# submarine0418/underwater_image_enhancement

Hardware: AMD Instinct MI355X
Metric: megapixels/sec enhanced (higher is better)
Workload: dtype f32/f64

## Files before the change

### include/uwie.h

```cpp
#ifndef UWIE_H_
#define UWIE_H_

#include <stddef.h>
#include <stdint.h>

#ifdef __cplusplus
extern "C" {
#endif

#define UWIE_OK 0
#define UWIE_E_INVALID (-1)
#define UWIE_E_WORKSPACE (-2)
#define UWIE_E_HIP (-3)
#define UWIE_E_NODEVICE (-4)
#define UWIE_E_DEVICE (-5)

#define UWIE_SURFACE_SIX 0
#define UWIE_SURFACE_DICT 1

#define UWIE_DICT_STRONG_DEHAZING 0
#define UWIE_DICT_MEDIUM_DEHAZING 1
#define UWIE_DICT_LIGHT_ENHANCEMENT 2
#define UWIE_DICT_CLAHE_ENHANCEMENT 3
#define UWIE_DICT_HISTOGRAM_EQUALIZATION 4
// ... 280 lines not shown
                           size_t workspace_bytes, void *stream);

int uwie_transmission_init(uwie_ctx *ctx, const uint8_t *d_in, const int32_t *d_kind, const float *d_A, int batch,
                           int H, int W, const uwie_params *p, float *d_t0, uint8_t *d_gray, void *stream);

int uwie_dark_patch_plan(int H, int W, int k, int *tile_w, int *tile_h);

int uwie_box_filter_f64(uwie_ctx *ctx, const double *d_src, double *d_dst, int batch, int H, int W, int ksize,
                        void *d_workspace, size_t workspace_bytes, void *stream);

int uwie_guided_filter(uwie_ctx *ctx, const uint8_t *d_gray, const float *d_t0, int batch, int H, int W, int ksize,
                       double eps, int exact, double *d_t, void *d_workspace, size_t workspace_bytes, void *stream);

int uwie_guided_plan(int batch, int H, int W, int ksize, int *split_row0, int *split_rows);

int uwie_guided_fill(int batch, int H, int W, int ksize, long long *items);

typedef struct uwie_clahe_plan_info {
    int32_t tile_w, tile_h, padded, clip_limit, wide_lut, nchunk, cells_walk, cells_flat;
} uwie_clahe_plan_info;
int uwie_clahe_plan(int batch, int H, int W, int tiles_x, int tiles_y, double clip_limit, int recomputed,
                    uwie_clahe_plan_info *out);

int uwie_restore(uwie_ctx *ctx, const uint8_t *d_in, const int32_t *d_kind, const float *d_A, const double *d_t,
                 int batch, int H, int W, float *d_out_f32, void *stream);

int uwie_percentiles_f32(uwie_ctx *ctx, const float *d_img, int batch, int H, int W, const double *q_percent, int nq,
                         float *d_out, void *d_workspace, size_t workspace_bytes, void *stream);

int uwie_percentiles_f64(uwie_ctx *ctx, const double *d_img, int batch, int H, int W, const double *q_percent, int nq,
                         double *d_out, void *d_workspace, size_t workspace_bytes, void *stream);

int uwie_stretch_f32(uwie_ctx *ctx, const float *d_img, float *d_out, int batch, int H, int W, double lo_percent,
                     double hi_percent, void *d_workspace, size_t workspace_bytes, void *stream);

int uwie_gamma_f32(uwie_ctx *ctx, const float *d_img, float *d_out, size_t n, double g, int mode, void *stream);

int uwie_clahe_f32(uwie_ctx *ctx, const float *d_img, float *d_out, int batch, int H, int W, double clip_limit,
                   int tiles_x, int tiles_y, void *d_workspace, size_t workspace_bytes, void *stream);

int uwie_rgb2gray_u8(uwie_ctx *ctx, const uint8_t *d_rgb, uint8_t *d_gray, size_t npixels, int gray_shift,
                     void *stream);
int uwie_rgb2lab_u8(uwie_ctx *ctx, const uint8_t *d_rgb, uint8_t *d_lab, size_t npixels, void *stream);
int uwie_lab2rgb_u8(uwie_ctx *ctx, const uint8_t *d_lab, uint8_t *d_rgb, size_t npixels, void *stream);
int uwie_clahe_u8(uwie_ctx *ctx, const uint8_t *d_plane, uint8_t *d_out, int batch, int H, int W, double clip_limit,
                  int tiles_x, int tiles_y, void *d_workspace, size_t workspace_bytes, void *stream);
// ... 10 lines not shown
```

### underwater_image_enhancement_amd/_lib.py

```python
from __future__ import annotations

import ctypes
import os
import subprocess

_HERE = os.path.dirname(os.path.abspath(__file__))
LIB_PATH = os.path.join(_HERE, "lib", "libuwie.so")
CSRC = os.path.join(_HERE, "csrc")

SURFACE_SIX, SURFACE_DICT = 0, 1
STATUS_DIFF_RANK = 16
STATUS_CLASSIFY_NAN = 64
LOSS_IDENTITY, LOSS_VGG, LOSS_GATED = 0, 1, 2
VGG_F32, VGG_F16, VGG_PARAMS = 0, 1, 1735488
PARAM_NET_PARAMS = {True: 8500100, False: 8459652}
MASKS_GIVEN, MASKS_DRAWN = 0, 1
TRAINER_PARAMS, TRAINER_GRADS, TRAINER_EXP_AVG, TRAINER_EXP_AVG_SQ = 0, 1, 2, 3
FLIP_LR, FLIP_UD = 1, 2
RESIZE_MAX_SIDE, RESIZE_MAX_SRC = 4096, 32768
INTER_F64, INTER_FX32, INTER_F32T = 0, 1, 2
DICT_STRATEGIES = {
    "strong_dehazing": 0,
    "medium_dehazing": 1,
    "light_enhancement": 2,
# ... 114 lines not shown
    "uwie_last_error": [],
    "uwie_version": [],
    "uwie_create": [_I, ctypes.POINTER(_VP)],
    "uwie_destroy": [_VP],
    "uwie_device_status": [_VP, _VP, ctypes.POINTER(ctypes.c_uint32)],
    "uwie_profile_enable": [_VP, _I],
    "uwie_profile_filter": [_VP, ctypes.c_char_p],
    "uwie_profile_collect": [_VP],
    "uwie_profile_row": [_VP, _I, ctypes.POINTER(ctypes.c_char_p), ctypes.POINTER(_D), ctypes.POINTER(_I)],
    "uwie_params_init": [_PP, _I, _I],
    "uwie_set_tuning": [_VP, ctypes.c_char_p, _I],
    "uwie_get_tuning": [_VP, ctypes.c_char_p, ctypes.POINTER(_I)],
    "uwie_workspace_bytes": [_I, _I, _I, _PP],
    "uwie_workspace_bytes_ctx": [_VP, _I, _I, _I, _PP],
    "uwie_workspace_bytes_all": [_I, _I, _I, _VP],
    "uwie_workspace_bytes_float": [_I, _I, _I, _PP, _I],
    "uwie_enhance_f32": [_VP, _VP, _VP, _VP, _VP, _I, _I, _I, _PP, _VP, _SZ, _VP],
    "uwie_enhance_f64": [_VP, _VP, _VP, _VP, _I, _I, _I, _PP, _VP, _SZ, _VP],
    "uwie_cast_classify_f32": [_VP, _VP, _I, _I, _I, _VP, _VP, _VP],
    "uwie_color_correct_f32": [_VP, _VP, _VP, _VP, _I, _I, _I, _VP],
    "uwie_guided_plan": [_I, _I, _I, _I, ctypes.POINTER(ctypes.c_int), ctypes.POINTER(ctypes.c_int)],
    "uwie_guided_fill": [_I, _I, _I, _I, ctypes.POINTER(ctypes.c_longlong)],
    "uwie_clahe_plan": [_I, _I, _I, _I, _I, _D, _I, ctypes.POINTER(UwieClahePlan)],
    "uwie_dark_patch_plan": [_I, _I, _I, ctypes.POINTER(ctypes.c_int), ctypes.POINTER(ctypes.c_int)],
    "uwie_enhance_u8": [_VP, _VP, _VP, _VP, _I, _I, _I, _PP, _VP, _SZ, _VP],
    "uwie_enhance_u8_f64": [_VP, _VP, _VP, _VP, _I, _I, _I, _PP, _VP, _SZ, _VP],
    "uwie_enhance_percentiles": [_VP, _VP, _SZ, _I, _I, _I, _PP, _VP, _VP],
    "uwie_enhance_all_u8": [_VP, _VP, _VP, _VP, _I, _I, _I, _VP, _VP, _SZ, _VP],
    "uwie_workspace_bytes_select": [_I, _I, _I, _VP, _I, _I],
    "uwie_select_best_u8": [_VP, _VP, _I, _I, _I, _VP, _I, _VP, _VP, _VP, _VP, _VP, _VP, _SZ, _VP],
    "uwie_workspace_bytes_underwater": [_I, _I, _I],
    "uwie_underwater_plan": [_I, _I, ctypes.POINTER(ctypes.c_int), ctypes.POINTER(ctypes.c_int)],
    "uwie_underwater_scores_u8": [_VP, _VP, _I, _I, _I, _I, _VP, _VP, _SZ, _VP],
    "uwie_workspace_bytes_reference": [_I, _I, _I],
    "uwie_reference_plan": [_I, _I, ctypes.POINTER(ctypes.c_int), ctypes.POINTER(ctypes.c_int)],
    "uwie_reference_scores_u8": [_VP, _VP, _VP, _I, _I, _I, _I, _I, _VP, _VP, _SZ, _VP],
    "uwie_workspace_bytes_gray_world": [_I, _I, _I],
    "uwie_gray_world_plan": [_I, _I, ctypes.POINTER(ctypes.c_int), ctypes.POINTER(ctypes.c_int)],
    "uwie_gray_world_u8": [_VP, _VP, _I, _I, _I, _D, _D, _D, _VP, _VP, _VP, _SZ, _VP],
    "uwie_workspace_bytes_fusion": [_I, _I, _I, _I],
    "uwie_fusion_plan": [_I, _I, _I, ctypes.POINTER(ctypes.c_int), ctypes.POINTER(ctypes.c_int)],
    "uwie_fusion_table": [_D, ctypes.POINTER(ctypes.c_uint8)],
    "uwie_fusion_u8": [_VP, _VP, _I, _I, _I, _D, _I, _I, _VP, _VP, _VP, _VP, _VP, _SZ, _VP],
    "uwie_pick_best_u8": [_VP, _VP, _I, _I, _I, _I, _VP, _I, _I, _VP, _VP, _VP],
    "uwie_diff_enhance_f32": [_VP, _VP, _VP, _I, _I, _I, _I, _VP, _I, _VP, _SZ, _VP],
    "uwie_diff_enhance_save_f32": [_VP, _VP, _VP, _I, _I, _I, _I, _VP, _I, _VP, _VP, _SZ, _VP],
# ... 134 lines not shown
```

### underwater_image_enhancement_amd/csrc/api.hip

```cpp
#include <algorithm>
#include <cmath>
#include <cstdarg>
#include <cstdio>
#include <cstring>
#include <type_traits>

#include "common.h"

#include <cstdlib>

namespace uwie {

static thread_local char g_err[512] = "";
static thread_local uwie_ctx *g_ctx = nullptr;
static const Tuning g_default_tuning{};

const Tuning &tune() { return g_ctx ? g_ctx->tune : g_default_tuning; }
uwie_ctx *current_ctx() { return g_ctx; }

void set_error(const char *fmt, ...)
{
    va_list ap;
    va_start(ap, fmt);
    vsnprintf(g_err, sizeof g_err, fmt, ap);
// ... 2016 lines not shown
    *items = g.route == GF_SPLIT ? guided_items(s, g) : 0;
    return UWIE_OK;
}

int uwie_dark_patch_plan(int H, int W, int k, int *tile_w, int *tile_h)
{
    UWIE_REQUIRE(tile_w && tile_h, "dark_patch_plan: NULL pointer");
    UWIE_CHECK_SHAPE(1, H, W);
    UWIE_REQUIRE(k >= 0 && k <= 31, "dark_patch_plan: dark_patch must be 0 .. 31");
    dark_patch_tile(tile_w, tile_h);
    return UWIE_OK;
}

int uwie_clahe_plan(int batch, int H, int W, int tiles_x, int tiles_y, double clip_limit, int recomputed,
                    uwie_clahe_plan_info *out)
{
    UWIE_REQUIRE(out, "clahe_plan: NULL pointer");
    UWIE_CHECK_SHAPE(batch, H, W);
    UWIE_REQUIRE(tiles_x >= 1 && tiles_y >= 1 && tiles_x * tiles_y <= 4096, "clahe_plan: bad tile grid");
    clahe_plan_info(Shape{batch, H, W}, clip_limit, tiles_x, tiles_y, recomputed != 0, out);
    return UWIE_OK;
}

int uwie_restore(uwie_ctx *ctx, const uint8_t *d_in, const int32_t *d_kind, const float *d_A, const double *d_t,
                 int batch, int H, int W, float *d_out_f32, void *stream)
{
    UWIE_REQUIRE(ctx && d_in && d_A && d_t && d_out_f32, "restore: NULL pointer");
    UWIE_SCOPE(ctx);
    UWIE_CHECK_SHAPE(batch, H, W);
    return launch_restore(d_in, d_kind, d_A, d_t, Shape{batch, H, W}, d_out_f32, (hipStream_t)stream);
}

int uwie_percentiles_f32(uwie_ctx *ctx, const float *d_img, int batch, int H, int W, const double *q_percent, int nq,
                         float *d_out, void *d_workspace, size_t workspace_bytes, void *stream)
{
    UWIE_REQUIRE(ctx && d_img && q_percent && d_out, "percentiles: NULL pointer");
    UWIE_SCOPE(ctx);
    UWIE_CHECK_SHAPE(batch, H, W);
    const Shape s{batch, H, W};
    UWIE_CHECK_WS(select_ws_bytes(s));
    return launch_percentiles(d_img, 0, s, q_percent, nq, d_out, d_workspace, (hipStream_t)stream);
}

int uwie_percentiles_f64(uwie_ctx *ctx, const double *d_img, int batch, int H, int W, const double *q_percent, int nq,
                         double *d_out, void *d_workspace, size_t workspace_bytes, void *stream)
{
// ... 129 lines not shown
```

### underwater_image_enhancement_amd/csrc/common.h

```cpp
#pragma once
#include <hip/hip_runtime.h>
#include <stddef.h>
#include <stdint.h>

#include "../../include/uwie.h"

namespace uwie {

void set_error(const char *fmt, ...);
#define UWIE_HIP_CHECK(expr)                                                            \
    do {                                                                                \
        hipError_t _e = (expr);                                                         \
        if (_e != hipSuccess) {                                                         \
            ::uwie::set_error("%s failed: %s (%s:%d)", #expr, hipGetErrorString(_e), __FILE__, __LINE__); \
            return UWIE_E_HIP;                                                          \
        }                                                                               \
    } while (0)
#define UWIE_LAUNCH_CHECK() UWIE_HIP_CHECK(hipGetLastError())
#define UWIE_REQUIRE(cond, msg)                 \
    do {                                        \
        if (!(cond)) {                          \
            ::uwie::set_error("%s", msg);       \
            return UWIE_E_INVALID;              \
        }                                       \
    } while (0)

constexpr int kCastBinadeMin = -2;
constexpr int kCastBinades = 34;

struct LabTables {
    uint16_t gamma[256];
    uint16_t cbrt[3072];
    int32_t fwd[9];
    uint8_t invgamma[4096];
    int32_t ltoyf[512];
    int32_t abtoxz[36864];
    int32_t inv[9];
};

struct CastTables {
    uint32_t R[kCastBinades][256];
    uint8_t tie[kCastBinades][256];
    uint32_t RT[256][kCastBinades];
    uint2 RT2[128][kCastBinades];
    uint8_t tiebin[256];
};

void build_lab_tables(LabTables *t);
void build_cast_tables(CastTables *t);

struct Profiler;
Profiler *prof_create();
void prof_destroy(Profiler *p);
void prof_enable(Profiler *p, bool on);
void prof_filter(Profiler *p, const char *name);
void prof_bind(Profiler *p);
int prof_collect(Profiler *p);
int prof_row(Profiler *p, int i, const char **name, double *ms, int *calls);
class ProfScope {
public:
// ... 457 lines not shown
```

### underwater_image_enhancement_amd/csrc/k_fused.hip

```cpp
#include <cstdlib>

#include "common.h"
#include "devutil.h"
#include "restore.h"

namespace uwie {

namespace {


typedef float f32x2 __attribute__((ext_vector_type(2)));
#ifndef UWIE_CLAHE_PREFETCH
#define UWIE_CLAHE_PREFETCH 0
#endif
#ifndef UWIE_STRETCH_WAVES
#define UWIE_STRETCH_WAVES 5
#endif
#define UWIE_DESCALE(x, n) (((x) + (1 << ((n)-1))) >> (n))

template <bool LIN, bool COLLECT, int NW = 2, typename V = float>
__global__ void __launch_bounds__(256) k_restore_planar_hist(RestoreSrc S, int npx, V *__restrict__ planar,
                                                             uint32_t *__restrict__ ghist, LinState *__restrict__ lin,
                                                             V *__restrict__ lists, uint32_t cap)
{
    constexpr int NB = LIN ? 2052 : 2048;
    constexpr bool F64 = sizeof(V) == 8;
    constexpr bool FAST = LIN && !F64;
    constexpr int NS = COLLECT ? 3 * NW : 1, SN = COLLECT ? (NW == 2 && !F64 ? 256 : 128) : 1;
    __shared__ uint32_t h[3][NB];
    __shared__ V stg[NS][SN];
    __shared__ uint32_t scount[NS], sbase[NS];
    __shared__ double dtab[FAST ? 768 : 1];
    const int b = blockIdx.y, tid = threadIdx.x;
    if (ghist) {
// ... 744 lines not shown
__device__ __forceinline__ int ab_to_xz(int i)
{
    const int t = __mul24(i, 108);
    const uint32_t tp = (uint32_t)(t + ((t >> 31) & 840) + 841 * 1100);
    const int lin = (int)__umulhi(tp, 5106980u) - (1100 + 290);
    const uint32_t sq = __umul24((uint32_t)i, (uint32_t)i) >> 14;
    const int cub = (int)(__umul24(sq, (uint32_t)i) >> 14);
    return i <= 3390 ? lin : cub;
}
__device__ __forceinline__ int ab_to_xz_cubic(int i)
{
    const uint32_t sq = __umul24((uint32_t)i, (uint32_t)i) >> 14;
    return (int)(__umul24(sq, (uint32_t)i) >> 14);
}

#define UWIE_APPLY_WALKS(gpr, rstep) ((gpr) <= 256 && (rstep) * (gpr) * 8 >= 256 * 7)
constexpr bool clahe_apply_walks(int gpr) { return UWIE_APPLY_WALKS(gpr, 256 / (gpr > 1 ? gpr : 1)); }
static_assert(clahe_apply_walks(1) && clahe_apply_walks(45) && clahe_apply_walks(85), "walk: narrow cells");
static_assert(!clahe_apply_walks(86) && !clahe_apply_walks(90) && !clahe_apply_walks(111), "flat: 341 .. 444 px");
static_assert(clahe_apply_walks(112) && clahe_apply_walks(128), "walk: 445 .. 512 px");
static_assert(!clahe_apply_walks(129) && !clahe_apply_walks(223), "flat: 513 .. 892 px");
static_assert(clahe_apply_walks(224) && clahe_apply_walks(256) && !clahe_apply_walks(257), "walk up to 1024 px, flat beyond");

template <bool CODES, bool F32OUT>
__global__ void __launch_bounds__(256) k_clahe_apply_out(const LabTables *__restrict__ T, const uint8_t *__restrict__ lab,
                                                         const uint8_t *__restrict__ lut, ClaheGeom g, int nchunk,
                                                         int gamma_mode, float gexp, const uint8_t *__restrict__ fin_code,
                                                         const float *__restrict__ fin_val, uint8_t *__restrict__ out_u8,
                                                         float *__restrict__ out_f32, uint8_t *__restrict__ codes_out,
                                                         uint32_t *__restrict__ hist)
{
    constexpr int NF = CODES ? 768 : 256;
    constexpr bool TWOSTEP = CODES || F32OUT;
    constexpr int BASE = 1 << 14;
    __shared__ __attribute__((aligned(16))) int s_l[256][4];
    __shared__ int s_l2[256];
    __shared__ uint8_t s_invgamma[TWOSTEP ? 4096 : 1];
    __shared__ uint8_t s_fin[TWOSTEP ? 1 : 4096];
    __shared__ float s_ff[NF];
    __shared__ uint8_t s_fu[NF];
    __shared__ uint32_t s_h[CODES ? 4 * 768 : 1];
    __shared__ uint32_t s_lut4[4][256];
    const int tid = threadIdx.x, b = blockIdx.y;
    const int cell = blockIdx.x / nchunk, chunk = blockIdx.x - cell * nchunk;
    const int cyi = cell / (g.tx + 1), cxi = cell - cyi * (g.tx + 1);
    const int cx0 = max(cxi * g.tw - g.tw / 2, 0), cx1 = min((cxi + 1) * g.tw - g.tw / 2, g.W);
    const int ry0 = max(cyi * g.th - g.th / 2, 0), ry1 = min((cyi + 1) * g.th - g.th / 2, g.H);
    const int rows_per = (ry1 - ry0 + nchunk - 1) / nchunk;
    const int cy0 = ry0 + chunk * rows_per, cy1 = min(cy0 + rows_per, ry1);
    if (cx0 >= cx1 || cy0 >= cy1) return;
    const int wx0 = min(max(cxi - 2, 0), max(g.tx - 4, 0)), wy0 = min(max(cyi - 2, 0), max(g.ty - 4, 0));
    const int m0 = T->inv[0], m1 = T->inv[1], m2 = T->inv[2], m3 = T->inv[3], m4 = T->inv[4], m5 = T->inv[5], m6 = T->inv[6],
              m7 = T->inv[7], m8 = T->inv[8];
    {
        const int yy = T->ltoyf[2 * tid], ify = T->ltoyf[2 * tid + 1];
        *reinterpret_cast<int4 *>(&s_l[tid][0]) = make_int4(ify - 128 * BASE / 500, ify + (128 * BASE / 200 - 1), m1 * yy + (1 << 13), m4 * yy + (1 << 13));
        s_l2[tid] = m7 * yy + (1 << 13);
    }
    if (TWOSTEP)
        for (int i = tid; i < 4096; i += 256) s_invgamma[i] = T->invgamma[i];
    if (CODES) {
        for (int i = tid; i < 768; i += 256) {
            s_fu[i] = fin_code ? fin_code[(size_t)b * 768 + i] : (uint8_t)0;
            s_ff[i] = fin_val ? fin_val[(size_t)b * 768 + i] : 0.f;
        }
        if (hist)
            for (int i = tid; i < 4 * 768; i += 256) s_h[i] = 0;
    } else {
        const float y = final_value(tid, gamma_mode, gexp);
        s_ff[tid] = y;
        s_fu[tid] = (uint8_t)quant_u8(y);
    }
    const uint8_t *Lt = lut + (size_t)b * g.tx * g.ty * 256;
    {
        const int wy = tid >> 6, q = tid & 63;
        const int tyy = min(wy0 + wy, g.ty - 1);
        uint32_t d[4];
#pragma unroll
        for (int wx = 0; wx < 4; ++wx)
            d[wx] = reinterpret_cast<const uint32_t *>(Lt + (size_t)(tyy * g.tx + min(wx0 + wx, g.tx - 1)) * 256)[q];
#pragma unroll
        for (int k = 0; k < 4; ++k)
            s_lut4[wy][4 * q + k] = ((d[0] >> (8 * k)) & 255u) | (((d[1] >> (8 * k)) & 255u) << 8) | (((d[2] >> (8 * k)) & 255u) << 16) |
                                    (((d[3] >> (8 * k)) & 255u) << 24);
    }
    __syncthreads();
    if (!TWOSTEP) {
        for (int i = tid; i < 1024; i += 256) {
            const uint32_t q = reinterpret_cast<const uint32_t *>(T->invgamma)[i];
            reinterpret_cast<uint32_t *>(s_fin)[i] = (uint32_t)s_fu[q & 255] | ((uint32_t)s_fu[(q >> 8) & 255] << 8) |
                                                     ((uint32_t)s_fu[(q >> 16) & 255] << 16) | ((uint32_t)s_fu[q >> 24] << 24);
        }
        __syncthreads();
    }
    const float inv_tw = 1.0f / (float)g.tw, inv_th = 1.0f / (float)g.th;
    const int gpr = (cx1 - cx0 + 3) / 4, total = (cy1 - cy0) * gpr;
    const uint32_t gmagic = (uint32_t)(((1ull << 32) + gpr - 1) / gpr);
    struct Cols {
        uint32_t sel[4];
        float xa[4], xa1[4];
    };
    auto cols_of = [&](int x0) {
        Cols C;
#pragma unroll
        for (int i = 0; i < 4; ++i) {
            const int x = min(x0 + i, g.W - 1);
            const float txf = (float)x * inv_tw - 0.5f;
            int tx1 = (int)floorf(txf);
            int tx2 = tx1 + 1;
            C.xa[i] = txf - (float)tx1;
            C.xa1[i] = 1.0f - C.xa[i];
            tx1 = max(tx1, 0);
            tx2 = min(tx2, g.tx - 1);
            const uint32_t c1 = (uint32_t)min(max(tx1 - wx0, 0), 3), c2 = (uint32_t)min(max(tx2 - wx0, 0), 3);
            C.sel[i] = c1 | ((4u + c1) << 8) | (c2 << 16) | ((4u + c2) << 24);
        }
        return C;
    };
    auto fetch = [&](int row, int xg, uint32_t (&w)[3]) {
        const int y = cy0 + row, x0 = cx0 + 4 * xg;
        if (row < cy1 - cy0 && x0 + 4 <= cx1) {
            const u32_unaligned *q = reinterpret_cast<const u32_unaligned *>(lab + (((size_t)b * g.H + y) * g.W + x0) * 3);
            w[0] = q[0]; w[1] = q[1]; w[2] = q[2];
        }
    };
    auto group = [&](int row, int xg, const Cols &C, const uint32_t (&pre)[3], bool has_pre) {
        const int y = cy0 + row, x0 = cx0 + 4 * xg, n = min(4, cx1 - x0);
        const size_t pix = ((size_t)b * g.H + y) * g.W + x0;
        Px4 in4;
        if (n == 4) {
            uint32_t w0 = pre[0], w1 = pre[1], w2 = pre[2];
            if (!has_pre) {
                const u32_unaligned *w = reinterpret_cast<const u32_unaligned *>(lab + pix * 3);
                w0 = w[0]; w1 = w[1]; w2 = w[2];
            }
            in4.r[0] = w0 & 255; in4.g[0] = (w0 >> 8) & 255; in4.b[0] = (w0 >> 16) & 255;
            in4.r[1] = w0 >> 24; in4.g[1] = w1 & 255; in4.b[1] = (w1 >> 8) & 255;
            in4.r[2] = (w1 >> 16) & 255; in4.g[2] = w1 >> 24; in4.b[2] = w2 & 255;
            in4.r[3] = (w2 >> 8) & 255; in4.g[3] = (w2 >> 16) & 255; in4.b[3] = w2 >> 24;
        } else {
            in4 = load_px4(lab + pix * 3, n, false);
        }
        const float tyf = (float)y * inv_th - 0.5f;
        int ty1 = (int)floorf(tyf);
        int ty2 = ty1 + 1;
        const float ya = tyf - (float)ty1, ya1 = 1.0f - ya;
        ty1 = max(ty1, 0);
        ty2 = min(ty2, g.ty - 1);
        const uint32_t *row1 = s_lut4[min(max(ty1 - wy0, 0), 3)], *row2 = s_lut4[min(max(ty2 - wy0, 0), 3)];
        const f32x2 yw = {ya1, ya};
        uint32_t o0[4], o1[4], o2[4];
        int ix[4], iz[4], yt0[4], yt1[4], yt2[4];
#pragma unroll
        for (int i = 0; i < 4; ++i) {
            const int v = in4.r[i], aa = in4.g[i], bb = in4.b[i];
            const uint32_t pk = __builtin_amdgcn_perm(row2[v], row1[v], C.sel[i]);
            const f32x2 l1 = {(float)(pk & 255u), (float)((pk >> 8) & 255u)};
            const f32x2 l2 = {(float)((pk >> 16) & 255u), (float)(pk >> 24)};
            const f32x2 rw = (l1 * C.xa1[i] + l2 * C.xa[i]) * yw;
            const float res = rw.x + rw.y;
            const int LL = min(max(__float2int_rn(res), 0), 255);
            const int4 ly = *reinterpret_cast<const int4 *>(&s_l[LL][0]);
            yt0[i] = ly.z;
            yt1[i] = ly.w;
// ... 10 lines not shown
            }
        } else {
#pragma unroll
            for (int i = 0; i < 4; ++i) {
                xx[i] = ab_to_xz(ix[i]);
                zz[i] = ab_to_xz(iz[i]);
            }
        }
#pragma unroll
        for (int i = 0; i < 4; ++i) {
            const int ro = min(max((__mul24(m0, xx[i]) + __mul24(m2, zz[i]) + yt0[i]) >> 14, 0), 4095);
            const int go = min(max((__mul24(m3, xx[i]) + __mul24(m5, zz[i]) + yt1[i]) >> 14, 0), 4095);
            const int bo = min(max((__mul24(m6, xx[i]) + __mul24(m8, zz[i]) + yt2[i]) >> 14, 0), 4095);
            if (TWOSTEP) {
                o0[i] = s_invgamma[ro];
                o1[i] = s_invgamma[go];
                o2[i] = s_invgamma[bo];
            } else {
                o0[i] = s_fin[ro];
                o1[i] = s_fin[go];
                o2[i] = s_fin[bo];
            }
        }
        const size_t o = pix * 3;
        if (CODES) {
            if (codes_out) {
                if (n == 4) {
                    u32_unaligned *w = reinterpret_cast<u32_unaligned *>(codes_out + o);
                    w[0] = o0[0] | (o1[0] << 8) | (o2[0] << 16) | (o0[1] << 24);
                    w[1] = o1[1] | (o2[1] << 8) | (o0[2] << 16) | (o1[2] << 24);
                    w[2] = o2[2] | (o0[3] << 8) | (o1[3] << 16) | (o2[3] << 24);
                } else {
                    store_px4(codes_out + o, o0, o1, o2, n, false);
                }
            }
#pragma unroll
            for (int i = 0; i < 4; ++i) {
                o1[i] += 256;
                o2[i] += 512;
            }
            if (hist) {
                uint32_t *hw = s_h + (tid >> 6) * 768;
                for (int i = 0; i < n; ++i) {
                    atomicAdd(&hw[o0[i]], 1u);
                    atomicAdd(&hw[o1[i]], 1u);
                    atomicAdd(&hw[o2[i]], 1u);
                }
            }
        }
        if (TWOSTEP && out_f32)
            for (int i = 0; i < n; ++i) {
                out_f32[o + 3 * i] = s_ff[o0[i]];
                out_f32[o + 3 * i + 1] = s_ff[o1[i]];
                out_f32[o + 3 * i + 2] = s_ff[o2[i]];
            }
        if (out_u8) {
            if (TWOSTEP) {
#pragma unroll
                for (int i = 0; i < 4; ++i) {
                    o0[i] = s_fu[o0[i]];
                    o1[i] = s_fu[o1[i]];
                    o2[i] = s_fu[o2[i]];
                }
            }
            if (n == 4) {
                u32_unaligned *w = reinterpret_cast<u32_unaligned *>(out_u8 + o);
                w[0] = o0[0] | (o1[0] << 8) | (o2[0] << 16) | (o0[1] << 24);
                w[1] = o1[1] | (o2[1] << 8) | (o0[2] << 16) | (o1[2] << 24);
                w[2] = o2[2] | (o0[3] << 8) | (o1[3] << 16) | (o2[3] << 24);
            } else {
                store_px4(out_u8 + o, o0, o1, o2, n, false);
            }
        }
    };
    const int rows = cy1 - cy0, rstep = 256 / max(gpr, 1);
    if (UWIE_APPLY_WALKS(gpr, rstep)) {
        if (tid < rstep * gpr) {
            const int xg = tid % gpr;
            const Cols C = cols_of(cx0 + 4 * xg);
#if UWIE_CLAHE_PREFETCH
            uint32_t nx[3] = {0, 0, 0};
            fetch(tid / gpr, xg, nx);
            for (int row = tid / gpr; row < rows; row += rstep) {
                const uint32_t cur[3] = {nx[0], nx[1], nx[2]};
                fetch(row + rstep, xg, nx);
                group(row, xg, C, cur, true);
            }
#else
            const uint32_t none[3] = {0, 0, 0};
            for (int row = tid / gpr; row < rows; row += rstep) group(row, xg, C, none, false);
#endif
        }
    } else {
        const uint32_t none[3] = {0, 0, 0};
        for (int gi = tid; gi < total; gi += 256) {
            const int row = gpr == 1 ? gi : (int)__umulhi((uint32_t)gi, gmagic), xg = gi - row * gpr;
            group(row, xg, cols_of(cx0 + 4 * xg), none, false);
        }
    }
    if (CODES && hist) {
        __syncthreads();
        for (int i = tid; i < 768; i += 256) {
            const uint32_t c = s_h[i] + s_h[768 + i] + s_h[2 * 768 + i] + s_h[3 * 768 + i];
            if (c) atomicAdd(&hist[(size_t)b * 768 + i], c);
        }
    }
}

__global__ void __launch_bounds__(256) k_stretch_out(const float *__restrict__ planar, const float *__restrict__ pct,
                                                     int pct_stride, float eps, int two, int npx, int gamma_mode, float gexp,
                                                     uint8_t *__restrict__ out_u8, float *__restrict__ out_f32)
{
    const int b = blockIdx.y;
    Stretch S;
    S.load(pct, b, pct_stride, eps, two);
    const float *r = planar + (size_t)b * 3 * npx;
    const bool aligned = (npx & 3) == 0;
    for (int p = (blockIdx.x * 256 + threadIdx.x) * 4; p < npx; p += gridDim.x * 1024) {
        const int n = min(4, npx - p);
        float v[3][4];
// ... 106 lines not shown
        const size_t o = ((size_t)b * npx + p) * 3;
        if (out_u8) store_px4(out_u8 + o, q[0], q[1], q[2], n, aligned);
        if (out_f32)
            for (int i = 0; i < n; ++i) {
                out_f32[o + 3 * i] = (float)f[0][i];
                out_f32[o + 3 * i + 1] = (float)f[1][i];
                out_f32[o + 3 * i + 2] = (float)f[2][i];
            }
        if (out_f64)
            for (int i = 0; i < n; ++i) {
                out_f64[o + 3 * i] = f[0][i];
                out_f64[o + 3 * i + 1] = f[1][i];
                out_f64[o + 3 * i + 2] = f[2][i];
            }
    }
}

struct ClaheLaunch {
    ClaheGeom g;
    bool padded;
    bool wide;
    int cells;
    int nchunk;
};

ClaheLaunch plan_clahe(Shape s, double clip, int tx, int ty, bool recomputed)
{
    ClaheLaunch L;
    ClaheGeom &g = L.g;
    g.H = s.H; g.W = s.W; g.tx = tx; g.ty = ty;
    int We = s.W, He = s.H;
    L.padded = s.W % tx != 0 || s.H % ty != 0;
    if (L.padded) {
        We = s.W + (tx - s.W % tx);
        He = s.H + (ty - s.H % ty);
    }
    g.tw = We / tx;
    g.th = He / ty;
    const int area = g.tw * g.th;
    g.lutScale = (float)(256 - 1) / (float)area;
    g.clip = 0;
    if (clip > 0.0) {
        g.clip = (int)(clip * area / 256);
        if (g.clip < 1) g.clip = 1;
    }
    L.wide = recomputed && (long)tx * ty * s.B < 512 && (long)g.tw * g.th >= 8192;
    L.cells = (tx + 1) * (ty + 1);
#ifndef UWIE_APPLY_TOTAL
#define UWIE_APPLY_TOTAL 25920
#endif
    const int nchunk = cdiv(UWIE_APPLY_TOTAL, L.cells * s.B);
    L.nchunk = std::max(1, std::min(nchunk, std::max(1, g.th / 16)));
    return L;
}

float gamma_exponent(int mode, double g) { return mode == 1 ? (float)g : mode == 2 ? (float)(1.0 / g) : 1.0f; }

int producer_blocks(int total, Shape s)
{
    const int nblk = std::min(std::max(cdiv(total, s.B), 16), 384);
    return std::min(nblk, cdiv((long long)s.npx(), 1024));
}

template <typename V>
struct HistRows;
template <>
struct HistRows<float> {
    static constexpr const char *collect = "k_restore_hist_collect", *collect4 = "k_restore_hist_collect4", *lin = "k_restore_hist_lin",
                                *key = "k_restore_hist_key", *plan_msg = "restore: a selection plan goes with its own linear histogram";
};
template <>
struct HistRows<double> {
    static constexpr const char *collect = "k_recover64_hist_collect", *collect4 = collect, *lin = "k_recover64_hist_lin",
                                *key = "k_recover64_hist_key", *plan_msg = "recover: a selection plan goes with its own linear histogram";
};
// ... 71 lines not shown
                    d_out_u8, d_out_f32, d_out_f64);
    else
        UWIE_LAUNCH(k_stretch64_out<false>, grid, dim3(256), 0, st, d_planar, RestoreSrc{}, d_pct, (int)s.npx(), apply_gamma,
                    1.0 / gamma, d_out_u8, d_out_f32, d_out_f64);
    UWIE_LAUNCH_CHECK();
    return UWIE_OK;
}

size_t tail_ws_bytes(Shape s, int tx, int ty)
{
    Carver c(nullptr);
    c.take<uint8_t>((size_t)s.B * tx * ty * 256);
    c.take<uint8_t>((size_t)s.B * s.npx() * 3);
    return c.total();
}

int launch_tail_clahe(uwie_ctx *ctx, const float *d_planar, const float *d_pct, int pct_stride, float eps, int two,
                      Shape s, double clip, int tx, int ty, int gamma_mode, double gamma, uint8_t *d_out_u8,
                      float *d_out_f32, void *ws, hipStream_t st, const RestoreSrc *src)
{
    Carver c(ws);
    uint8_t *lut = c.take<uint8_t>((size_t)s.B * tx * ty * 256);
    uint8_t *lab = c.take<uint8_t>((size_t)s.B * s.npx() * 3);
    const ClaheLaunch L = plan_clahe(s, clip, tx, ty, src != nullptr);
    const ClaheGeom &g = L.g;
    const auto k_stretch_lab_lut_wide = k_stretch_lab_lut<1, 1024>;
    if (L.wide)
        UWIE_LAUNCH(k_stretch_lab_lut_wide, dim3(tx * ty, s.B), dim3(1024), 0, st, ctx->d_lab, d_planar, *src, d_pct, pct_stride,
                    eps, two, (const uint8_t *)nullptr, g, lab, lut);
    else if (src)
        UWIE_LAUNCH(k_stretch_lab_lut<1>, dim3(tx * ty, s.B), dim3(256), 0, st, ctx->d_lab, d_planar, *src, d_pct, pct_stride,
                    eps, two, (const uint8_t *)nullptr, g, lab, lut);
    else
        UWIE_LAUNCH(k_stretch_lab_lut<0>, dim3(tx * ty, s.B), dim3(256), 0, st, ctx->d_lab, d_planar, RestoreSrc{}, d_pct,
                    pct_stride, eps, two, (const uint8_t *)nullptr, g, lab, lut);
    UWIE_LAUNCH_CHECK();
    const int cells = L.cells, nchunk = L.nchunk;
    const auto k_clahe_apply_u8 = k_clahe_apply_out<false, false>;
    const auto k_clahe_apply_f32 = k_clahe_apply_out<false, true>;
    if (d_out_f32)
        UWIE_LAUNCH(k_clahe_apply_f32, dim3(cells * nchunk, s.B), dim3(256), 0, st, ctx->d_lab, lab, lut, g, nchunk, gamma_mode,
                    gamma_exponent(gamma_mode, gamma), (const uint8_t *)nullptr, (const float *)nullptr, d_out_u8, d_out_f32,
                    (uint8_t *)nullptr, (uint32_t *)nullptr);
    else
        UWIE_LAUNCH(k_clahe_apply_u8, dim3(cells * nchunk, s.B), dim3(256), 0, st, ctx->d_lab, lab, lut, g, nchunk, gamma_mode,
                    gamma_exponent(gamma_mode, gamma), (const uint8_t *)nullptr, (const float *)nullptr, d_out_u8, d_out_f32,
                    (uint8_t *)nullptr, (uint32_t *)nullptr);
    UWIE_LAUNCH_CHECK();
    return UWIE_OK;
}

int launch_clahe_apply_codes(uwie_ctx *ctx, const uint8_t *d_lab, const uint8_t *d_tile_lut, Shape s, double clip, int tx,
                             int ty, const uint8_t *d_fin_code, const float *d_fin_val, uint8_t *d_out_u8, float *d_out_f32,
                             uint8_t *d_codes_out, uint32_t *d_hist, hipStream_t st)
{
    const ClaheLaunch L = plan_clahe(s, clip, tx, ty, false);
    const ClaheGeom &g = L.g;
    const int cells = L.cells, nchunk = L.nchunk;
    const auto k_clahe_apply_codes = k_clahe_apply_out<true, false>;
    UWIE_LAUNCH(k_clahe_apply_codes, dim3(cells * nchunk, s.B), dim3(256), 0, st, ctx->d_lab, d_lab, d_tile_lut, g, nchunk, 0, 1.0f,
                d_fin_code, d_fin_val, d_out_u8, d_out_f32, d_codes_out, d_hist);
    UWIE_LAUNCH_CHECK();
    return UWIE_OK;
}

int launch_codes_lab_lut(uwie_ctx *ctx, const uint8_t *d_in, const uint8_t *d_code_lut, Shape s, double clip, int tx, int ty,
                         uint8_t *d_lab, uint8_t *d_tile_lut, hipStream_t st)
{
    const ClaheGeom g = plan_clahe(s, clip, tx, ty, false).g;
    RestoreSrc src{};
    src.in = d_in;
    UWIE_LAUNCH(k_stretch_lab_lut<2>, dim3(tx * ty, s.B), dim3(256), 0, st, ctx->d_lab, (const float *)nullptr, src,
                (const float *)nullptr, 0, 0.0f, 0, d_code_lut, g, d_lab, d_tile_lut);
    UWIE_LAUNCH_CHECK();
    return UWIE_OK;
}

int launch_tail_plain(const float *d_planar, const float *d_pct, int pct_stride, float eps, int two, Shape s,
                      int gamma_mode, double gamma, uint8_t *d_out_u8, float *d_out_f32, hipStream_t st)
{
    UWIE_LAUNCH(k_stretch_out, dim3(grid_for(s.npx(), 4096), s.B), dim3(256), 0, st, d_planar, d_pct, pct_stride, eps, two,
                (int)s.npx(), gamma_mode, gamma_exponent(gamma_mode, gamma), d_out_u8, d_out_f32);
    UWIE_LAUNCH_CHECK();
// ... 5 lines not shown
```

### underwater_image_enhancement_amd/csrc/tables.cpp

```cpp
#include <cmath>
#include <cstring>

#include "common.h"

namespace uwie {

namespace {

float cv_cube_root(float value)
{
    uint32_t bits;
    std::memcpy(&bits, &value, 4);
    const uint32_t mag = bits & 0x7fffffffu, sign = bits & 0x80000000u;
    if (mag == 0) return value;
    int ex = int(mag >> 23) - 127;
    int shx = ex % 3;
    if (shx >= 0) shx -= 3;
    ex = (ex - shx) / 3;
    uint32_t fb = (mag & 0x7fffffu) | (uint32_t(shx + 127) << 23);
    float frf;
    std::memcpy(&frf, &fb, 4);
    const double f = frf;
    const double num = ((((45.2548339756803022511987494 * f + 192.2798368355061050458134625) * f +
                          119.1654824285581628956914143) * f + 13.43250139086239872172837314) * f +
// ... 44 lines not shown
        const float f = x < thresh ? std::fmaf(x, slope, bias) : cv_cube_root(x);
        t->cbrt[i] = (uint16_t)std::lrintf(float(1 << kLabShift2) * f);
    }
    for (int i = 0; i < 256; ++i) {
        int y, ify;
        if (i <= 20) {
            y = (int)std::lrintf(float(i * kBase * 20 * 9) / float(17 * 29 * 29 * 29));
            ify = (int)std::lrintf(float(kBase) * (16.0f / 116.0f + float(i * 100) / float(4 * 255 * 29)));
        } else {
            const float fy = float(i * 100 * kBase) / float(255 * 116) + float(16 * kBase) / 116.0f;
            ify = (int)std::lrintf(fy);
            y = (int)std::lrintf(fy * fy * fy / float(kBase * kBase));
        }
        t->ltoyf[2 * i] = y;
        t->ltoyf[2 * i + 1] = ify;
    }
    for (int i = kMinAB; i < kBase * 9 / 4 + kMinAB; ++i)
        t->abtoxz[i - kMinAB] = i <= 3390 ? i * 108 / 841 - kBase * 16 / 116 * 108 / 841 : i * i / kBase * i / kBase;
    for (int r = 0; r < 3; ++r)
        for (int c = 0; c < 3; ++c) {
            t->fwd[r * 3 + c] = (int)std::lrint(double(1 << kLabShift) * rgb2xyz[r * 3 + c] / white[r]);
            t->inv[r * 3 + c] = (int)std::lrint(double(1 << kLabShift) * xyz2rgb[r * 3 + c] * white[c]);
        }
}

void build_cast_tables(CastTables *t)
{
    for (int k = 0; k < 256; ++k) {
        const float x = float(k) / 255.0f;
        uint32_t bits;
        std::memcpy(&bits, &x, 4);
        const uint64_t M = k ? ((bits & 0x7fffffu) | 0x800000u) : 0;
        const int E = int(bits >> 23) - 127 - 23;
        for (int ei = 0; ei < kCastBinades; ++ei) {
            const int shift = (kCastBinadeMin + ei - 23) - E;
            uint64_t R = 0;
            uint8_t tie = 0;
            if (M == 0) {
            } else if (shift <= 0) {
                R = M << (-shift);
            } else if (shift < 40) {
                const uint64_t half = 1ull << (shift - 1), rem = M & ((1ull << shift) - 1);
                R = M >> shift;
                if (rem > half) R += 1;
                else if (rem == half) tie = 1;
            }
// ... 20 lines not shown
```

Baseline: 59540.

## Precompute CLAHE apply per-class geometry and Lab tables on host

The CLAHE apply kernel now receives a host-precomputed ClaheApply struct holding per-edge-class rows_per, groups-per-row, walk step and magic divisors, and it uses a 3D grid (cell x, cell y, batch) so the cell index no longer comes from integer division. The Lab inverse tables are precomputed into LabTables on the host instead of per block. For gamma_mode 0 in u8 mode the final table copy is loaded directly, skipping one sync. Addressing switches to 32-bit byte offsets per frame, which adds a guard that rejects frames of 2^32 bytes or more. The goal is to cut per-block setup and integer-division overhead in the apply kernel.

```diff
diff --git a/include/uwie.h b/include/uwie.h
--- a/include/uwie.h
+++ b/include/uwie.h
@@ -326,6 +326,8 @@
 int uwie_clahe_plan(int batch, int H, int W, int tiles_x, int tiles_y, double clip_limit, int recomputed,
                     uwie_clahe_plan_info *out);
 
+int uwie_clahe_apply_tables(int32_t *ltoyf, int32_t *inv, int32_t *l4, int32_t *l2);
+
 int uwie_restore(uwie_ctx *ctx, const uint8_t *d_in, const int32_t *d_kind, const float *d_A, const double *d_t,
                  int batch, int H, int W, float *d_out_f32, void *stream);
 
diff --git a/underwater_image_enhancement_amd/_lib.py b/underwater_image_enhancement_amd/_lib.py
--- a/underwater_image_enhancement_amd/_lib.py
+++ b/underwater_image_enhancement_amd/_lib.py
@@ -160,6 +160,7 @@
     "uwie_guided_plan": [_I, _I, _I, _I, ctypes.POINTER(ctypes.c_int), ctypes.POINTER(ctypes.c_int)],
     "uwie_guided_fill": [_I, _I, _I, _I, ctypes.POINTER(ctypes.c_longlong)],
     "uwie_clahe_plan": [_I, _I, _I, _I, _I, _D, _I, ctypes.POINTER(UwieClahePlan)],
+    "uwie_clahe_apply_tables": [_VP, _VP, _VP, _VP],
     "uwie_dark_patch_plan": [_I, _I, _I, ctypes.POINTER(ctypes.c_int), ctypes.POINTER(ctypes.c_int)],
     "uwie_enhance_u8": [_VP, _VP, _VP, _VP, _I, _I, _I, _PP, _VP, _SZ, _VP],
     "uwie_enhance_u8_f64": [_VP, _VP, _VP, _VP, _I, _I, _I, _PP, _VP, _SZ, _VP],
diff --git a/underwater_image_enhancement_amd/csrc/api.hip b/underwater_image_enhancement_amd/csrc/api.hip
--- a/underwater_image_enhancement_amd/csrc/api.hip
+++ b/underwater_image_enhancement_amd/csrc/api.hip
@@ -2062,6 +2062,18 @@
     return UWIE_OK;
 }
 
+int uwie_clahe_apply_tables(int32_t *ltoyf, int32_t *inv, int32_t *l4, int32_t *l2)
+{
+    LabTables *t = new LabTables();
+    build_lab_tables(t);
+    if (ltoyf) memcpy(ltoyf, t->ltoyf, sizeof(t->ltoyf));
+    if (inv) memcpy(inv, t->inv, sizeof(t->inv));
+    if (l4) memcpy(l4, t->apply_l, sizeof(t->apply_l));
+    if (l2) memcpy(l2, t->apply_l2, sizeof(t->apply_l2));
+    delete t;
+    return UWIE_OK;
+}
+
 int uwie_restore(uwie_ctx *ctx, const uint8_t *d_in, const int32_t *d_kind, const float *d_A, const double *d_t,
                  int batch, int H, int W, float *d_out_f32, void *stream)
 {
diff --git a/underwater_image_enhancement_amd/csrc/common.h b/underwater_image_enhancement_amd/csrc/common.h
--- a/underwater_image_enhancement_amd/csrc/common.h
+++ b/underwater_image_enhancement_amd/csrc/common.h
@@ -36,6 +36,8 @@
     int32_t ltoyf[512];
     int32_t abtoxz[36864];
     int32_t inv[9];
+    alignas(16) int32_t apply_l[256][4];
+    int32_t apply_l2[256];
 };
 
 struct CastTables {
diff --git a/underwater_image_enhancement_amd/csrc/k_fused.hip b/underwater_image_enhancement_amd/csrc/k_fused.hip
--- a/underwater_image_enhancement_amd/csrc/k_fused.hip
+++ b/underwater_image_enhancement_amd/csrc/k_fused.hip
@@ -10,6 +10,9 @@
 
 
 typedef float f32x2 __attribute__((ext_vector_type(2)));
+#ifndef UWIE_APPLY_SETUP_ONLY
+#define UWIE_APPLY_SETUP_ONLY 0
+#endif
 #ifndef UWIE_CLAHE_PREFETCH
 #define UWIE_CLAHE_PREFETCH 0
 #endif
@@ -800,9 +803,25 @@
 static_assert(!clahe_apply_walks(129) && !clahe_apply_walks(223), "flat: 513 .. 892 px");
 static_assert(clahe_apply_walks(224) && clahe_apply_walks(256) && !clahe_apply_walks(257), "walk up to 1024 px, flat beyond");
 
+struct ApplyCols {
+    int gpr;
+    int rstep;
+    uint32_t gmagic;
+    uint32_t tmagic;
+};
+struct ClaheApply {
+    ClaheGeom g;
+    int nchunk;
+    uint32_t cmagic;
+    int rows_per[3];
+    float inv_tw, inv_th;
+    ApplyCols col[3];
+};
+#define UWIE_APPLY_CLASS(i, hi, size) ((i) == 0 ? 0 : (hi) <= (size) ? 1 : 2)
+
 template <bool CODES, bool F32OUT>
 __global__ void __launch_bounds__(256) k_clahe_apply_out(const LabTables *__restrict__ T, const uint8_t *__restrict__ lab,
-                                                         const uint8_t *__restrict__ lut, ClaheGeom g, int nchunk,
+                                                         const uint8_t *__restrict__ lut, ClaheApply A,
                                                          int gamma_mode, float gexp, const uint8_t *__restrict__ fin_code,
                                                          const float *__restrict__ fin_val, uint8_t *__restrict__ out_u8,
                                                          float *__restrict__ out_f32, uint8_t *__restrict__ codes_out,
@@ -810,7 +829,6 @@
 {
     constexpr int NF = CODES ? 768 : 256;
     constexpr bool TWOSTEP = CODES || F32OUT;
-    constexpr int BASE = 1 << 14;
     __shared__ __attribute__((aligned(16))) int s_l[256][4];
     __shared__ int s_l2[256];
     __shared__ uint8_t s_invgamma[TWOSTEP ? 4096 : 1];
@@ -819,22 +837,21 @@
     __shared__ uint8_t s_fu[NF];
     __shared__ uint32_t s_h[CODES ? 4 * 768 : 1];
     __shared__ uint32_t s_lut4[4][256];
-    const int tid = threadIdx.x, b = blockIdx.y;
-    const int cell = blockIdx.x / nchunk, chunk = blockIdx.x - cell * nchunk;
-    const int cyi = cell / (g.tx + 1), cxi = cell - cyi * (g.tx + 1);
-    const int cx0 = max(cxi * g.tw - g.tw / 2, 0), cx1 = min((cxi + 1) * g.tw - g.tw / 2, g.W);
-    const int ry0 = max(cyi * g.th - g.th / 2, 0), ry1 = min((cyi + 1) * g.th - g.th / 2, g.H);
-    const int rows_per = (ry1 - ry0 + nchunk - 1) / nchunk;
+    const ClaheGeom &g = A.g;
+    const int tid = threadIdx.x, b = blockIdx.z, cyi = blockIdx.y, nchunk = A.nchunk;
+    const int cxi = nchunk == 1 ? (int)blockIdx.x : (int)__umulhi(blockIdx.x, A.cmagic), chunk = blockIdx.x - cxi * nchunk;
+    const int nx1 = (cxi + 1) * g.tw - g.tw / 2, ny1 = (cyi + 1) * g.th - g.th / 2;
+    const int cx0 = max(nx1 - g.tw, 0), cx1 = min(nx1, g.W);
+    const int ry0 = max(ny1 - g.th, 0), ry1 = min(ny1, g.H);
+    const int rcls = UWIE_APPLY_CLASS(cyi, ny1, g.H), rows_per = rcls == 0 ? A.rows_per[0] : rcls == 1 ? A.rows_per[1] : A.rows_per[2];
     const int cy0 = ry0 + chunk * rows_per, cy1 = min(cy0 + rows_per, ry1);
     if (cx0 >= cx1 || cy0 >= cy1) return;
+    const int ccls = UWIE_APPLY_CLASS(cxi, nx1, g.W);
+    const ApplyCols P = ccls == 0 ? A.col[0] : ccls == 1 ? A.col[1] : A.col[2];
     const int wx0 = min(max(cxi - 2, 0), max(g.tx - 4, 0)), wy0 = min(max(cyi - 2, 0), max(g.ty - 4, 0));
-    const int m0 = T->inv[0], m1 = T->inv[1], m2 = T->inv[2], m3 = T->inv[3], m4 = T->inv[4], m5 = T->inv[5], m6 = T->inv[6],
-              m7 = T->inv[7], m8 = T->inv[8];
-    {
-        const int yy = T->ltoyf[2 * tid], ify = T->ltoyf[2 * tid + 1];
-        *reinterpret_cast<int4 *>(&s_l[tid][0]) = make_int4(ify - 128 * BASE / 500, ify + (128 * BASE / 200 - 1), m1 * yy + (1 << 13), m4 * yy + (1 << 13));
-        s_l2[tid] = m7 * yy + (1 << 13);
-    }
+    const int m0 = T->inv[0], m2 = T->inv[2], m3 = T->inv[3], m5 = T->inv[5], m6 = T->inv[6], m8 = T->inv[8];
+    *reinterpret_cast<int4 *>(&s_l[tid][0]) = *reinterpret_cast<const int4 *>(&T->apply_l[tid][0]);
+    s_l2[tid] = T->apply_l2[tid];
     if (TWOSTEP)
         for (int i = tid; i < 4096; i += 256) s_invgamma[i] = T->invgamma[i];
     if (CODES) {
@@ -844,10 +861,13 @@
         }
         if (hist)
             for (int i = tid; i < 4 * 768; i += 256) s_h[i] = 0;
-    } else {
+    } else if (TWOSTEP || gamma_mode != 0) {
         const float y = final_value(tid, gamma_mode, gexp);
         s_ff[tid] = y;
         s_fu[tid] = (uint8_t)quant_u8(y);
+    } else {
+        for (int i = tid; i < 1024; i += 256)
+            reinterpret_cast<uint32_t *>(s_fin)[i] = reinterpret_cast<const uint32_t *>(T->invgamma)[i];
     }
     const uint8_t *Lt = lut + (size_t)b * g.tx * g.ty * 256;
     {
@@ -863,7 +883,7 @@
                                     (((d[3] >> (8 * k)) & 255u) << 24);
     }
     __syncthreads();
-    if (!TWOSTEP) {
+    if (!TWOSTEP && gamma_mode != 0) {
         for (int i = tid; i < 1024; i += 256) {
             const uint32_t q = reinterpret_cast<const uint32_t *>(T->invgamma)[i];
             reinterpret_cast<uint32_t *>(s_fin)[i] = (uint32_t)s_fu[q & 255] | ((uint32_t)s_fu[(q >> 8) & 255] << 8) |
@@ -871,9 +891,8 @@
         }
         __syncthreads();
     }
-    const float inv_tw = 1.0f / (float)g.tw, inv_th = 1.0f / (float)g.th;
-    const int gpr = (cx1 - cx0 + 3) / 4, total = (cy1 - cy0) * gpr;
-    const uint32_t gmagic = (uint32_t)(((1ull << 32) + gpr - 1) / gpr);
+    const float inv_tw = A.inv_tw, inv_th = A.inv_th;
+    const int gpr = P.gpr, total = (cy1 - cy0) * gpr;
     struct Cols {
         uint32_t sel[4];
         float xa[4], xa1[4];
@@ -895,21 +914,22 @@
         }
         return C;
     };
-    auto fetch = [&](int row, int xg, uint32_t (&w)[3]) {
-        const int y = cy0 + row, x0 = cx0 + 4 * xg;
-        if (row < cy1 - cy0 && x0 + 4 <= cx1) {
-            const u32_unaligned *q = reinterpret_cast<const u32_unaligned *>(lab + (((size_t)b * g.H + y) * g.W + x0) * 3);
+    const size_t img = (size_t)b * ((size_t)g.H * g.W * 3);
+    const uint8_t *lab_b = lab + img;
+    uint8_t *out_u8_b = out_u8 + img, *codes_b = codes_out + img;
+    float *out_f32_b = out_f32 + img;
+    auto fetch = [&](int y, int n, uint32_t o, uint32_t (&w)[3]) {
+        if (y < cy1 && n == 4) {
+            const u32_unaligned *q = reinterpret_cast<const u32_unaligned *>(lab_b + o);
             w[0] = q[0]; w[1] = q[1]; w[2] = q[2];
         }
     };
-    auto group = [&](int row, int xg, const Cols &C, const uint32_t (&pre)[3], bool has_pre) {
-        const int y = cy0 + row, x0 = cx0 + 4 * xg, n = min(4, cx1 - x0);
-        const size_t pix = ((size_t)b * g.H + y) * g.W + x0;
+    auto group = [&](int y, int n, uint32_t o, const Cols &C, const uint32_t (&pre)[3], bool has_pre) {
         Px4 in4;
         if (n == 4) {
             uint32_t w0 = pre[0], w1 = pre[1], w2 = pre[2];
             if (!has_pre) {
-                const u32_unaligned *w = reinterpret_cast<const u32_unaligned *>(lab + pix * 3);
+                const u32_unaligned *w = reinterpret_cast<const u32_unaligned *>(lab_b + o);
                 w0 = w[0]; w1 = w[1]; w2 = w[2];
             }
             in4.r[0] = w0 & 255; in4.g[0] = (w0 >> 8) & 255; in4.b[0] = (w0 >> 16) & 255;
@@ -917,7 +937,7 @@
             in4.r[2] = (w1 >> 16) & 255; in4.g[2] = w1 >> 24; in4.b[2] = w2 & 255;
             in4.r[3] = (w2 >> 8) & 255; in4.g[3] = (w2 >> 16) & 255; in4.b[3] = w2 >> 24;
         } else {
-            in4 = load_px4(lab + pix * 3, n, false);
+            in4 = load_px4(lab_b + o, n, false);
         }
         const float tyf = (float)y * inv_th - 0.5f;
         int ty1 = (int)floorf(tyf);
@@ -974,16 +994,15 @@
                 o2[i] = s_fin[bo];
             }
         }
-        const size_t o = pix * 3;
         if (CODES) {
             if (codes_out) {
                 if (n == 4) {
-                    u32_unaligned *w = reinterpret_cast<u32_unaligned *>(codes_out + o);
+                    u32_unaligned *w = reinterpret_cast<u32_unaligned *>(codes_b + o);
                     w[0] = o0[0] | (o1[0] << 8) | (o2[0] << 16) | (o0[1] << 24);
                     w[1] = o1[1] | (o2[1] << 8) | (o0[2] << 16) | (o1[2] << 24);
                     w[2] = o2[2] | (o0[3] << 8) | (o1[3] << 16) | (o2[3] << 24);
                 } else {
-                    store_px4(codes_out + o, o0, o1, o2, n, false);
+                    store_px4(codes_b + o, o0, o1, o2, n, false);
                 }
             }
 #pragma unroll
@@ -993,6 +1012,7 @@
             }
             if (hist) {
                 uint32_t *hw = s_h + (tid >> 6) * 768;
+#pragma nounroll
                 for (int i = 0; i < n; ++i) {
                     atomicAdd(&hw[o0[i]], 1u);
                     atomicAdd(&hw[o1[i]], 1u);
@@ -1000,12 +1020,15 @@
                 }
             }
         }
-        if (TWOSTEP && out_f32)
+        if (TWOSTEP && out_f32) {
+            float *f = reinterpret_cast<float *>(reinterpret_cast<char *>(out_f32_b) + o * 4u);
+#pragma nounroll
             for (int i = 0; i < n; ++i) {
-                out_f32[o + 3 * i] = s_ff[o0[i]];
-                out_f32[o + 3 * i + 1] = s_ff[o1[i]];
-                out_f32[o + 3 * i + 2] = s_ff[o2[i]];
-            }
+                f[3 * i] = s_ff[o0[i]];
+                f[3 * i + 1] = s_ff[o1[i]];
+                f[3 * i + 2] = s_ff[o2[i]];
+            }
+        }
         if (out_u8) {
             if (TWOSTEP) {
 #pragma unroll
@@ -1016,38 +1039,46 @@
                 }
             }
             if (n == 4) {
-                u32_unaligned *w = reinterpret_cast<u32_unaligned *>(out_u8 + o);
+                u32_unaligned *w = reinterpret_cast<u32_unaligned *>(out_u8_b + o);
                 w[0] = o0[0] | (o1[0] << 8) | (o2[0] << 16) | (o0[1] << 24);
                 w[1] = o1[1] | (o2[1] << 8) | (o0[2] << 16) | (o1[2] << 24);
                 w[2] = o2[2] | (o0[3] << 8) | (o1[3] << 16) | (o2[3] << 24);
             } else {
-                store_px4(out_u8 + o, o0, o1, o2, n, false);
+                store_px4(out_u8_b + o, o0, o1, o2, n, false);
             }
         }
     };
-    const int rows = cy1 - cy0, rstep = 256 / max(gpr, 1);
-    if (UWIE_APPLY_WALKS(gpr, rstep)) {
+    const int rstep = P.rstep;
+#if UWIE_APPLY_SETUP_ONLY
+    if (gexp == 1.0f) return;
+#endif
+    if (rstep > 0) {
         if (tid < rstep * gpr) {
-            const int xg = tid % gpr;
-            const Cols C = cols_of(cx0 + 4 * xg);
+            const int row0 = (int)(__umul24((uint32_t)tid, P.tmagic) >> 16), xg = tid - (int)__umul24((uint32_t)row0, (uint32_t)gpr);
+            const int x0 = cx0 + 4 * xg, n = min(4, cx1 - x0);
+            const Cols C = cols_of(x0);
+            uint32_t o = (uint32_t)((cy0 + row0) * g.W + x0) * 3u;
+            const uint32_t ostep = (uint32_t)(rstep * g.W) * 3u;
 #if UWIE_CLAHE_PREFETCH
             uint32_t nx[3] = {0, 0, 0};
-            fetch(tid / gpr, xg, nx);
-            for (int row = tid / gpr; row < rows; row += rstep) {
+            fetch(cy0 + row0, n, o, nx);
+            for (int y = cy0 + row0; y < cy1; y += rstep, o += ostep) {
                 const uint32_t cur[3] = {nx[0], nx[1], nx[2]};
-                fetch(row + rstep, xg, nx);
-                group(row, xg, C, cur, true);
+                fetch(y + rstep, n, o + ostep, nx);
+                group(y, n, o, C, cur, true);
             }
 #else
             const uint32_t none[3] = {0, 0, 0};
-            for (int row = tid / gpr; row < rows; row += rstep) group(row, xg, C, none, false);
+            for (int y = cy0 + row0; y < cy1; y += rstep, o += ostep) group(y, n, o, C, none, false);
 #endif
         }
     } else {
         const uint32_t none[3] = {0, 0, 0};
+        const uint32_t gmagic = P.gmagic;
         for (int gi = tid; gi < total; gi += 256) {
             const int row = gpr == 1 ? gi : (int)__umulhi((uint32_t)gi, gmagic), xg = gi - row * gpr;
-            group(row, xg, cols_of(cx0 + 4 * xg), none, false);
+            const int y = cy0 + row, x0 = cx0 + 4 * xg;
+            group(y, min(4, cx1 - x0), (uint32_t)(y * g.W + x0) * 3u, cols_of(x0), none, false);
         }
     }
     if (CODES && hist) {
@@ -1200,7 +1231,18 @@
     bool wide;
     int cells;
     int nchunk;
+    ClaheApply a;
+    dim3 apply_grid(int B) const { return dim3((g.tx + 1) * nchunk, g.ty + 1, B); }
 };
+
+int apply_class_extent(int k, int t, int n, int size)
+{
+    if (k == 0) return std::min(t - t / 2, size);
+    if (k == 1) return t;
+    for (int i = 1; i <= n; ++i)
+        if ((i + 1) * t - t / 2 > size) return std::max(size - (i * t - t / 2), 0);
+    return 0;
+}
 
 ClaheLaunch plan_clahe(Shape s, double clip, int tx, int ty, bool recomputed)
 {
@@ -1229,6 +1271,20 @@
 #endif
     const int nchunk = cdiv(UWIE_APPLY_TOTAL, L.cells * s.B);
     L.nchunk = std::max(1, std::min(nchunk, std::max(1, g.th / 16)));
+    ClaheApply &a = L.a;
+    a.g = g;
+    a.nchunk = L.nchunk;
+    a.cmagic = (uint32_t)(((1ull << 32) + L.nchunk - 1) / L.nchunk);
+    a.inv_tw = 1.0f / (float)g.tw;
+    a.inv_th = 1.0f / (float)g.th;
+    for (int k = 0; k < 3; ++k) {
+        a.rows_per[k] = cdiv(apply_class_extent(k, g.th, ty, s.H), L.nchunk);
+        ApplyCols &c = a.col[k];
+        c.gpr = std::max((apply_class_extent(k, g.tw, tx, s.W) + 3) / 4, 1);
+        c.rstep = clahe_apply_walks(c.gpr) ? 256 / c.gpr : 0;
+        c.gmagic = (uint32_t)(((1ull << 32) + c.gpr - 1) / c.gpr);
+        c.tmagic = (uint32_t)(((1u << 16) + c.gpr - 1) / c.gpr);
+    }
     return L;
 }
 
@@ -1346,6 +1402,7 @@
     Carver c(ws);
     uint8_t *lut = c.take<uint8_t>((size_t)s.B * tx * ty * 256);
     uint8_t *lab = c.take<uint8_t>((size_t)s.B * s.npx() * 3);
+    UWIE_REQUIRE((unsigned long long)s.npx() * 3 * (d_out_f32 ? 4 : 1) < (1ull << 32), "CLAHE tail: a frame's output plane must stay below 2^32 bytes");
     const ClaheLaunch L = plan_clahe(s, clip, tx, ty, src != nullptr);
     const ClaheGeom &g = L.g;
     const auto k_stretch_lab_lut_wide = k_stretch_lab_lut<1, 1024>;
@@ -1359,15 +1416,14 @@
         UWIE_LAUNCH(k_stretch_lab_lut<0>, dim3(tx * ty, s.B), dim3(256), 0, st, ctx->d_lab, d_planar, RestoreSrc{}, d_pct,
                     pct_stride, eps, two, (const uint8_t *)nullptr, g, lab, lut);
     UWIE_LAUNCH_CHECK();
-    const int cells = L.cells, nchunk = L.nchunk;
     const auto k_clahe_apply_u8 = k_clahe_apply_out<false, false>;
     const auto k_clahe_apply_f32 = k_clahe_apply_out<false, true>;
     if (d_out_f32)
-        UWIE_LAUNCH(k_clahe_apply_f32, dim3(cells * nchunk, s.B), dim3(256), 0, st, ctx->d_lab, lab, lut, g, nchunk, gamma_mode,
+        UWIE_LAUNCH(k_clahe_apply_f32, L.apply_grid(s.B), dim3(256), 0, st, ctx->d_lab, lab, lut, L.a, gamma_mode,
                     gamma_exponent(gamma_mode, gamma), (const uint8_t *)nullptr, (const float *)nullptr, d_out_u8, d_out_f32,
                     (uint8_t *)nullptr, (uint32_t *)nullptr);
     else
-        UWIE_LAUNCH(k_clahe_apply_u8, dim3(cells * nchunk, s.B), dim3(256), 0, st, ctx->d_lab, lab, lut, g, nchunk, gamma_mode,
+        UWIE_LAUNCH(k_clahe_apply_u8, L.apply_grid(s.B), dim3(256), 0, st, ctx->d_lab, lab, lut, L.a, gamma_mode,
                     gamma_exponent(gamma_mode, gamma), (const uint8_t *)nullptr, (const float *)nullptr, d_out_u8, d_out_f32,
                     (uint8_t *)nullptr, (uint32_t *)nullptr);
     UWIE_LAUNCH_CHECK();
@@ -1378,11 +1434,10 @@
                              int ty, const uint8_t *d_fin_code, const float *d_fin_val, uint8_t *d_out_u8, float *d_out_f32,
                              uint8_t *d_codes_out, uint32_t *d_hist, hipStream_t st)
 {
+    UWIE_REQUIRE((unsigned long long)s.npx() * 3 * (d_out_f32 ? 4 : 1) < (1ull << 32), "CLAHE tail: a frame's output plane must stay below 2^32 bytes");
     const ClaheLaunch L = plan_clahe(s, clip, tx, ty, false);
-    const ClaheGeom &g = L.g;
-    const int cells = L.cells, nchunk = L.nchunk;
     const auto k_clahe_apply_codes = k_clahe_apply_out<true, false>;
-    UWIE_LAUNCH(k_clahe_apply_codes, dim3(cells * nchunk, s.B), dim3(256), 0, st, ctx->d_lab, d_lab, d_tile_lut, g, nchunk, 0, 1.0f,
+    UWIE_LAUNCH(k_clahe_apply_codes, L.apply_grid(s.B), dim3(256), 0, st, ctx->d_lab, d_lab, d_tile_lut, L.a, 0, 1.0f,
                 d_fin_code, d_fin_val, d_out_u8, d_out_f32, d_codes_out, d_hist);
     UWIE_LAUNCH_CHECK();
     return UWIE_OK;
diff --git a/underwater_image_enhancement_amd/csrc/tables.cpp b/underwater_image_enhancement_amd/csrc/tables.cpp
--- a/underwater_image_enhancement_amd/csrc/tables.cpp
+++ b/underwater_image_enhancement_amd/csrc/tables.cpp
@@ -90,6 +90,14 @@
             t->fwd[r * 3 + c] = (int)std::lrint(double(1 << kLabShift) * rgb2xyz[r * 3 + c] / white[r]);
             t->inv[r * 3 + c] = (int)std::lrint(double(1 << kLabShift) * xyz2rgb[r * 3 + c] * white[c]);
         }
+    for (int i = 0; i < 256; ++i) {
+        const int y = t->ltoyf[2 * i], ify = t->ltoyf[2 * i + 1];
+        t->apply_l[i][0] = ify - 128 * kBase / 500;
+        t->apply_l[i][1] = ify + (128 * kBase / 200 - 1);
+        t->apply_l[i][2] = t->inv[1] * y + (1 << 13);
+        t->apply_l[i][3] = t->inv[4] * y + (1 << 13);
+        t->apply_l2[i] = t->inv[7] * y + (1 << 13);
+    }
 }
 
 void build_cast_tables(CastTables *t)
```

After: 59250. Within noise of the previous version (-0.5%).
